# ironmanaudi/GNN-decode

Hardware: AMD Instinct MI355X
Metric: codewords/sec (whole node) at matched BER, T-iter GNN decode (higher is better)
Workload: dtype f32; 1 GPU; bch_63_45 cgnni decode, T=25, batch=65536/GPU; code=bch_63_45, model=cgnni, iters=25, global_batch=65536, parallelism=dp1 (codeword shards)

## Files before the change

### gnn-decode_amd/csrc/gnnd_common.h

```cpp
#pragma once
#include <hip/hip_runtime.h>
#include <stdint.h>
#include <math.h>
#include "../../include/gnnd.h"

#ifndef GNND_BLOCK
#define GNND_BLOCK 256
#endif

#ifdef GNND_TUNING
#include <stdlib.h>
#define gnnd_tune_env(name) getenv(name)
#else
#define gnnd_tune_env(name) ((const char*)nullptr)
#endif

enum GnndDebugBit {
    GNND_DBG_LDS_POS = 0,
    GNND_DBG_VAR = 1,
    GNND_DBG_SLOT = 2,
    GNND_DBG_NODE = 3,
    GNND_DBG_GRID = 4,
};
#ifdef GNND_DEBUG
// ... 64 lines not shown
#define GNND_PMARK(pf, i) pf.mark(i)
#define GNND_PREPORT(pf, tag, n, iters) pf.report(tag, n, iters)
#define GNND_PARG(pf, i) , &pf, i
#else
#define GNND_PPROF(pf) do { } while (0)
#define GNND_PSTART(pf, on) do { } while (0)
#define GNND_PMARK(pf, i) do { } while (0)
#define GNND_PREPORT(pf, tag, n, iters) do { } while (0)
#define GNND_PARG(pf, i)
#endif

struct GraphView {
    int V, C, E, N;
    int max_dv, max_dc;
    const uint32_t* edge_vc;
    const int* var_ptr;
    const int* chk_ptr;
    const int* chk_edge;
    int G, logG, R;
    int padded;
    int padr;
    const uint32_t* slot;
    const int* vslot;
    const uint32_t* slot_ve;
    const uint2* var_ord;
    const uint2* vlay;
    int vgroup, spare, P1;
    int ts;
    int xs, xv0, xc0, os, o0, es, e0;
};
#define GNND_SLOT_PAD 0x80000000u

struct gnnd_graph {
    GraphView view;
    GraphView rview;
    GraphView pview;
    GraphView rlay[7];
    GraphView rlayx[7];
    void* dev;
    size_t table_bytes;
    int ncomp;
    gnnd_graph* comp[8];
    GraphView* dcomp;
    int nosplit;
    int min_dc;
    int nlayers, max_layer;
    int* layer_dev;
    int* layer_of;
    int uf_nvert;
    int* uf_dev;
    int* uf_ends;
};
constexpr int kMaxComp = 8;

__host__ __device__ inline int graph_table_ints(int V, int C, int E) {
    return E + (V + 1) + (C + 1) + E;
}

int set_hip_error(hipError_t e);

#define GNND_HIP_CHECK(call)                                   \
    do {                                                       \
        hipError_t _e = (call);                                \
        if (_e != hipSuccess) return set_hip_error(_e);        \
    } while (0)

#define GNND_LAUNCH_CHECK()                                    \
    do {                                                       \
        hipError_t _e = hipGetLastError();                     \
        if (_e != hipSuccess) return set_hip_error(_e);        \
    } while (0)

struct FastDiv {
    uint32_t d, m, s;
};
inline FastDiv make_fastdiv(uint32_t d) {
    FastDiv f;
    f.d = d;
    uint32_t l = 0;
    while ((1u << l) < d) ++l;
    f.s = l;
    f.m = (uint32_t)((((uint64_t)1 << 32) * (((uint64_t)1 << l) - d)) / d + 1);
    return f;
}
__device__ __forceinline__ uint32_t fdiv(uint32_t n, const FastDiv& f) {
    return (__umulhi(n, f.m) + n) >> f.s;
}

__device__ __forceinline__ float g_tanh(float x) { return tanhf(x); }
__device__ __forceinline__ float g_log(float x) { return logf(x); }
__device__ __forceinline__ float g_exp(float x) { return expf(x); }
__device__ __forceinline__ float g_log1p(float x) { return log1pf(x); }
__device__ __forceinline__ double g_log1p(double x) { return log1p(x); }
__device__ __forceinline__ float g_cos(float x) { return cosf(x); }
__device__ __forceinline__ double g_cos(double x) { return cos(x); }
__device__ __forceinline__ float g_abs(float x) { return fabsf(x); }
__device__ __forceinline__ double g_abs(double x) { return fabs(x); }
template <typename T> __device__ __forceinline__ T g_fma(T a, T b, T c) { return fma(a, b, c); }
template <typename T> __device__ __forceinline__ T g_min(T a, T b) { return a < b ? a : b; }
template <typename T> __device__ __forceinline__ T g_max(T a, T b) { return a > b ? a : b; }
template <typename T> __device__ __forceinline__ T g_clamp(T x, T lo, T hi) {
    return x < lo ? lo : (x > hi ? hi : x);
}

__constant__ static const double kSpCoef[23] = {
    1.0 / 6227020800.0, 1.0 / 479001600.0, 1.0 / 39916800.0, 1.0 / 3628800.0,
// ... 2712 lines not shown
```

### gnn-decode_amd/csrc/gnnd_graph.hip

```cpp
#include "gnnd_common.h"
#include "gnnd_minsum_layered_host.h"
#include "gnnd_uf_host.h"
#include <stdlib.h>
#include <string.h>
#include <vector>
#include <algorithm>
#include <cmath>
#include <cstdio>

static thread_local int g_last_hip_error = 0;

int set_hip_error(hipError_t e) {
    g_last_hip_error = (int)e;
    return GNND_ERR_HIP;
}

extern "C" int gnnd_last_hip_error(void) { return g_last_hip_error; }

GNND_DEBUG_TU(graph)

extern "C" int gnnd_version(void) { return GNND_VERSION; }

extern "C" const char* gnnd_status_string(int s) {
    switch (s) {
        case GNND_OK: return "ok";
        case GNND_ERR_INVALID_ARG: return "invalid argument";
        case GNND_ERR_HIP: return "HIP runtime error";
        case GNND_ERR_UNSUPPORTED: return "unsupported configuration";
        case GNND_ERR_GRAPH: return "invalid Tanner graph (edges must be unique and sorted by (v, c))";
        case GNND_ERR_ALLOC: return "device allocation failed";
        default: return "unknown status";
    }
}

namespace {

struct SlotPlan {
    int G = 0, R = 0, padded = 0, padr = 0;
    std::vector<uint32_t> slot, slot_ve;
    std::vector<int> vslot;
};
struct Layout {
    bool ok = false;
    int P = 0;
    std::vector<int> vlay, slot;
    int ts = 0;
    std::vector<int> tpos;
};
struct HostTables {
    int V = 0, C = 0, E = 0, max_dv = 0, max_dc = 0, min_dc = 0, nints = 0, ord_off = 0, nsr = 0;
    int plan_off[3] = {0, 0, 0};
    SlotPlan plans[3];
    Layout lays[7], laysx[7];
    int lay_off[7] = {0}, layx_off[7] = {0};
    std::vector<int> table;
};

bool slot_spread_disabled() {
    static bool v = [] {
        const char* e = gnnd_tune_env("GNND_NO_SLOT_SPREAD");
        return e && e[0] == '1';
    }();
    return v;
}

void spread_check_slots(int C, int G, int R, int cw, int P, const std::vector<int>& cdeg,
                        std::vector<int>& slot) {
    const int GR = G * R, P1 = (P + 1) | 1;
    const long items = (long)C * cw * G;
    const int nh = (int)((items + 31) / 32);
    if (nh <= 0 || cw < 1) return;
    std::vector<std::vector<int>> cr_groups((size_t)C * R);
    for (int h = 0; h < nh; ++h) {
        int last = -1;
        for (int f = 32 * h; f < 32 * h + 32 && f < items; ++f) {
            const int c = (f / G) / cw;
            if (c == last) continue;
            last = c;
            for (int r = 0; r < R; ++r) cr_groups[(size_t)c * R + r].push_back(h * R + r);
        }
    }
    auto group_cost = [&](int grp) {
        const int h = grp / R, r = grp % R;
        int addr[32], n = 0;
        for (int f = 32 * h; f < 32 * h + 32 && f < items; ++f) {
            const int gi = f / G, g = f % G, c = gi / cw, b = gi % cw;
            const int k = g * R + r;
            const int pos = k < cdeg[c] ? (int)((uint32_t)slot[(size_t)c * GR + k] >> 16) : P;
            const int a = b * P1 + pos;
            bool dup = false;
            for (int i = 0; i < n && !dup; ++i) dup = addr[i] == a;
            if (!dup) addr[n++] = a;
        }
        int cnt[32] = {0}, m = 0;
        for (int i = 0; i < n; ++i) m = std::max(m, ++cnt[addr[i] & 31]);
        return m;
    };
// ... 130 lines not shown
        std::vector<int> touched, nc;
        for (long it = 0; it < iters; ++it) {
            const int a = (int)rnd(V);
            const int p2 = (int)rnd(ts);
            const int b = pos_owner[p2];
            if (b == a) continue;
            const int pa = tp[a];
            tp[a] = p2;
            if (b >= 0) tp[b] = pa;
            touched.clear();
            for (int q : of_var[a]) touched.push_back(q);
            if (b >= 0) for (int q : of_var[b]) touched.push_back(q);
            std::sort(touched.begin(), touched.end());
            touched.erase(std::unique(touched.begin(), touched.end()), touched.end());
            long delta = 0;
            nc.resize(touched.size());
            for (size_t i = 0; i < touched.size(); ++i) {
                nc[i] = cost_of(touched[i], ts, tp);
                delta += nc[i] - gc[touched[i]];
            }
            const double temp = 2.0 * (1.0 - (double)it / iters) + 0.05;
            const double u = (double)rnd(1u << 30) / (double)(1u << 30);
            if (delta <= 0 || u < exp(-(double)delta / temp)) {
                for (size_t i = 0; i < touched.size(); ++i) gc[touched[i]] = nc[i];
                cur += delta;
                pos_owner[p2] = a;
                pos_owner[pa] = b;
                if (cur < bestc) { bestc = cur; best = tp; }
            } else {
                tp[a] = pa;
                if (b >= 0) tp[b] = p2;
            }
        }
        if (best_total < 0 || bestc < best_total) {
            best_total = bestc;
            ts_out = ts;
            tpos_out = best;
        }
    }
    static const bool log = [] {
        const char* e = gnnd_tune_env("GNND_SLOT_SPREAD_LOG");
        return e && e[0] == '1';
    }();
    if (log) {
        std::vector<int> id(V);
        for (int v = 0; v < V; ++v) id[v] = v;
        long c0 = 0;
        for (int q = 0; q < ng; ++q) c0 += cost_of(q, V, id);
        fprintf(stderr, "gnnd t rows: C=%d G=%d R=%d cw=%d gather+write cycles per tile iteration "
                        "%ld (ts = V) -> %ld (ts = %d)\n", C, G, R, cw, c0, best_total, ts_out);
    }
}

int build_tables(const int64_t* h_var, const int64_t* h_chk, int64_t num_edges, int32_t V,
                 int32_t C, HostTables& T) {
    if (!h_var || !h_chk || num_edges <= 0 || V <= 0 || C <= 0) return GNND_ERR_INVALID_ARG;
    if (V > 65535 || C > 65535 || num_edges > 65535) return GNND_ERR_UNSUPPORTED;
    const int E = (int)num_edges;
    std::vector<uint32_t> evc(E);
    std::vector<int> vptr(V + 1, 0), cptr(C + 1, 0), cedge(E);
    for (int e = 0; e < E; ++e) {
        int64_t v = h_var[e], c = h_chk[e];
        if (v < 0 || v >= V || c < 0 || c >= C) return GNND_ERR_GRAPH;
        if (e > 0) {
            int64_t pv = h_var[e - 1], pc = h_chk[e - 1];
            if (v < pv || (v == pv && c <= pc)) return GNND_ERR_GRAPH;
        }
        evc[e] = (uint32_t)v | ((uint32_t)c << 16);
        vptr[v + 1]++;
        cptr[c + 1]++;
    }
    int max_dv = 0, max_dc = 0;
    for (int v = 0; v < V; ++v) { max_dv = vptr[v + 1] > max_dv ? vptr[v + 1] : max_dv; vptr[v + 1] += vptr[v]; }
    int min_dc = C > 0 ? cptr[1] : 0;
    for (int c = 0; c < C; ++c) {
        max_dc = cptr[c + 1] > max_dc ? cptr[c + 1] : max_dc;
        min_dc = cptr[c + 1] < min_dc ? cptr[c + 1] : min_dc;
        cptr[c + 1] += cptr[c];
    }
    {
        std::vector<int> fill(cptr.begin(), cptr.end() - 1);
        for (int e = 0; e < E; ++e) cedge[fill[h_chk[e]]++] = e;
    }
    static const int force_r = [] {
        const char* e = gnnd_tune_env("GNND_GROUP_R");
        return e ? atoi(e) : 0;
    }();
    auto build_plan = [&](int pref, SlotPlan& sp) -> bool {
        long best = -1;
        for (int R = 1; R <= 4; ++R) {
            int need = (max_dc + R - 1) / R, G = 1;
            while (G < need) G <<= 1;
            if (G > 64) continue;
            long slots = (long)C * G * R;
            if (force_r == R) { best = slots; sp.G = G; sp.R = R; break; }
            const bool tie_wins = pref == 1 || (pref == 2 && R == 2);
            if (best < 0 || slots < best || (tie_wins && slots == best)) {
                best = slots; sp.G = G; sp.R = R;
            }
        }
        if (best < 0) return false;
        const int ns = C * sp.G * sp.R;
        sp.slot.assign(ns, GNND_SLOT_PAD);
        sp.slot_ve.assign(ns, (uint32_t)E << 16);
        sp.vslot.assign(E, 0);
        sp.padded = 0;
        for (int c = 0; c < C; ++c) {
            sp.padded |= (cptr[c + 1] - cptr[c]) != sp.G * sp.R;
            sp.padr = std::max(sp.padr, std::min(sp.R, sp.G * sp.R - (cptr[c + 1] - cptr[c])));
            for (int k = cptr[c], i = 0; k < cptr[c + 1]; ++k, ++i) {
                int e = cedge[k];
                int pos = c * sp.G * sp.R + i;
                sp.slot[pos] = evc[e] & 0xffffu;
                sp.slot_ve[pos] = (evc[e] & 0xffffu) | ((uint32_t)e << 16);
                sp.vslot[e] = pos;
            }
        }
        return true;
    };
    SlotPlan* plans = T.plans;
    for (int i = 0; i < 3; ++i)
        if (!build_plan(i, plans[i])) return GNND_ERR_UNSUPPORTED;

    std::vector<int> vord(V);
    for (int v = 0; v < V; ++v) vord[v] = v;
    std::stable_sort(vord.begin(), vord.end(), [&](int a, int b) {
        return vptr[a + 1] - vptr[a] < vptr[b + 1] - vptr[b];
    });

    const int nints = graph_table_ints(V, C, E);
    int* plan_off = T.plan_off;
    int off = nints;
    for (int i = 0; i < 3; ++i) {
        plan_off[i] = off;
        off += 2 * (int)plans[i].slot.size() + E;
    }
    const int ord_off = (off + 1) & ~1;
    const int nsr = (int)plans[1].slot.size();
    auto build_layout = [&](int gs, bool with_x, Layout& L) {
        std::vector<int> epos(E);
        L.vlay.assign(2 * V, 0);
        int pos = 0;
        for (int j0 = 0; j0 < V; j0 += gs) {
            const int j1 = std::min(V, j0 + gs);
            int dpad = 0;
            for (int j = j0; j < j1; ++j) dpad = std::max(dpad, vptr[vord[j] + 1] - vptr[vord[j]]);
            if (with_x) ++dpad;
            for (int j = j0; j < j1; ++j) {
                const int v = vord[j];
                L.vlay[2 * j] = v | (dpad << 16);
                L.vlay[2 * j + 1] = pos;
                for (int e = vptr[v]; e < vptr[v + 1]; ++e) epos[e] = pos + (e - vptr[v]);
                pos += dpad;
            }
        }
        L.P = pos;
        if (pos >= 65535) return;
        L.ok = true;
        L.slot.assign(nsr, pos << 16);
        for (int k = 0; k < nsr; ++k) {
            const uint32_t sv = plans[1].slot_ve[k];
            const int e = (int)(sv >> 16);
            if (e < E) L.slot[k] = (int)(sv & 0xffffu) | (epos[e] << 16);
        }
        const bool tile_ok = (long)(64 / gs) * C * plans[1].G <= 12L * 256;
        if (with_x && gs >= 2 && gs <= 32 && plans[1].G <= 16 && tile_ok && !slot_spread_disabled()) {
            std::vector<int> cdeg(C);
            for (int c = 0; c < C; ++c) cdeg[c] = cptr[c + 1] - cptr[c];
            spread_check_slots(C, plans[1].G, plans[1].R, 64 / gs, pos, cdeg, L.slot);
        }
        L.ts = V;
        L.tpos.resize(V);
        for (int v = 0; v < V; ++v) L.tpos[v] = v;
        if (with_x && gs >= 2 && gs <= 32 && plans[1].G <= 16 && tile_ok && !tperm_disabled()) {
            std::vector<int> cdeg(C), vo(V);
            for (int c = 0; c < C; ++c) cdeg[c] = cptr[c + 1] - cptr[c];
            for (int j = 0; j < V; ++j) vo[j] = L.vlay[2 * j] & 0xffff;
            place_t_rows(C, plans[1].G, plans[1].R, 64 / gs, V, vo, cdeg, L.slot, L.ts, L.tpos);
        }
        if (with_x) {
            for (int j = 0; j < V; ++j) L.vlay[2 * j + 1] |= L.tpos[L.vlay[2 * j] & 0xffff] << 16;
            for (int k = 0; k < nsr; ++k)
                L.slot[k] = (L.slot[k] & ~0xffff) | L.tpos[L.slot[k] & 0xffff];
        }
    };
    Layout* lays = T.lays;
    Layout* laysx = T.laysx;
    int* lay_off = T.lay_off;
    int* layx_off = T.layx_off;
    off = ord_off + 2 * V;
    for (int i = 0; i < 7; ++i) {
        for (int x = 0; x < 2; ++x) {
            if (i == 0 && !x) continue;
            Layout& L = x ? laysx[i] : lays[i];
            build_layout(1 << i, x != 0, L);
            if (!L.ok) continue;
            (x ? layx_off : lay_off)[i] = off;
            off = (off + 2 * V + nsr + 1) & ~1;
        }
    }
    std::vector<int>& table = T.table;
    table.assign(off, 0);
    memcpy(table.data(), evc.data(), sizeof(int) * E);
    memcpy(table.data() + E, vptr.data(), sizeof(int) * (V + 1));
    memcpy(table.data() + E + V + 1, cptr.data(), sizeof(int) * (C + 1));
    memcpy(table.data() + E + V + 1 + C + 1, cedge.data(), sizeof(int) * E);
    for (int i = 0; i < 3; ++i) {
        const int ns = (int)plans[i].slot.size();
        memcpy(table.data() + plan_off[i], plans[i].slot.data(), sizeof(int) * ns);
        memcpy(table.data() + plan_off[i] + ns, plans[i].vslot.data(), sizeof(int) * E);
        memcpy(table.data() + plan_off[i] + ns + E, plans[i].slot_ve.data(), sizeof(int) * ns);
    }
    for (int i = 0; i < V; ++i) {
        const int v = vord[i];
        table[ord_off + 2 * i] = v | ((vptr[v + 1] - vptr[v]) << 16);
        table[ord_off + 2 * i + 1] = vptr[v];
    }
    for (int i = 0; i < 7; ++i)
        for (int x = 0; x < 2; ++x) {
            const Layout& L = x ? laysx[i] : lays[i];
            if (!L.ok) continue;
            const int o = (x ? layx_off : lay_off)[i];
            memcpy(table.data() + o, L.vlay.data(), sizeof(int) * 2 * V);
            memcpy(table.data() + o + 2 * V, L.slot.data(), sizeof(int) * nsr);
        }

    T.V = V; T.C = C; T.E = E; T.max_dv = max_dv; T.max_dc = max_dc; T.min_dc = min_dc;
    T.nints = nints; T.ord_off = ord_off; T.nsr = nsr;
    return GNND_OK;
}

int check_tables(const HostTables& T, int32_t* report) {
    const int E = T.E, V = T.V, C = T.C;
    const std::vector<int>& t = T.table;
    const int* vptr = t.data() + E;
    const int* cptr = vptr + V + 1;
    const int* cedge = cptr + C + 1;
    int fails = 0, nlay = 0;
    for (int p = 0; p < 3; ++p) {
        const SlotPlan& sp = T.plans[p];
        const int GR = sp.G * sp.R;
        if ((int)sp.slot_ve.size() != C * GR) { ++fails; continue; }
        for (int c = 0; c < C; ++c) {
            const int deg = cptr[c + 1] - cptr[c];
            if (deg > GR) ++fails;
            for (int i = 0; i < GR; ++i) {
                const int e = (int)(sp.slot_ve[c * GR + i] >> 16);
                if (i < deg) {
                    if (e != cedge[cptr[c] + i] || sp.vslot[e] != c * GR + i) ++fails;
                    if ((int)(sp.slot_ve[c * GR + i] & 0xffffu) != (int)(t[e] & 0xffff)) ++fails;
                } else if (e != E) {
                    ++fails;
                }
            }
            for (int gi = 0; gi < sp.G; ++gi) {
                int pad = 0;
                for (int r = 0; r < sp.R; ++r) {
                    const bool isp = (int)(sp.slot_ve[c * GR + gi * sp.R + r] >> 16) == E;
                    if (!isp && pad) ++fails;
                    pad += isp;
                }
                if (pad > sp.padr) ++fails;
            }
        }
    }
    for (int x = 0; x < 2; ++x)
        for (int i = x ? 0 : 1; i < 7; ++i) {
            const Layout& L = x ? T.laysx[i] : T.lays[i];
            if (!L.ok) continue;
            ++nlay;
            std::vector<int> owner(L.P + 1, -1), epos(E, -1);
            int expect = 0;
            const bool tx = x != 0;
            const int ts = tx ? L.ts : V;
            if (tx) {
                std::vector<int> used(ts > 0 ? ts : 1, 0);
                if ((int)L.tpos.size() != V || ts < V || ts > 65535) ++fails;
                else
                    for (int v = 0; v < V; ++v)
                        if (L.tpos[v] < 0 || L.tpos[v] >= ts || used[L.tpos[v]]++) ++fails;
            }
            auto tp = [&](int v) { return tx && (int)L.tpos.size() == V ? L.tpos[v] : v; };
            for (int j = 0; j < V; ++j) {
                const int v = L.vlay[2 * j] & 0xffff, dpad = (int)((uint32_t)L.vlay[2 * j] >> 16);
                const int pos = L.vlay[2 * j + 1] & 0xffff;
                if (((uint32_t)L.vlay[2 * j + 1] >> 16) != (uint32_t)(tx ? tp(v) : 0)) ++fails;
                const int deg = vptr[v + 1] - vptr[v];
                if (pos != expect || dpad < deg + x || pos + dpad > L.P) { ++fails; continue; }
                expect = pos + dpad;
                for (int k = 0; k < dpad; ++k) {
                    if (owner[pos + k] != -1) ++fails;
                    owner[pos + k] = v;
                }
                for (int e = vptr[v]; e < vptr[v + 1]; ++e) epos[e] = pos + (e - vptr[v]);
            }
            if (expect != L.P) ++fails;
            const SlotPlan& sp = T.plans[1];
            const int GR = sp.G * sp.R;
            std::vector<int> epos_inv(L.P + 1, -1), seen(E, 0);
            for (int e = 0; e < E; ++e)
                if (epos[e] >= 0) epos_inv[epos[e]] = e;
            for (int c = 0; c < C; ++c) {
                const int deg = cptr[c + 1] - cptr[c];
                for (int k = 0; k < GR; ++k) {
                    const uint32_t sl = (uint32_t)L.slot[c * GR + k];
                    const int pos = (int)(sl >> 16);
                    if (k >= deg) {
                        if (pos != L.P) ++fails;
                        continue;
                    }
                    const int e = pos <= L.P ? epos_inv[pos] : -1;
                    if (e < 0 || (int)(t[e] >> 16) != c || (int)(sl & 0xffffu) != tp((int)(t[e] & 0xffff)) ||
                        seen[e]++)
                        ++fails;
                }
            }
        }
    if (report) {
        report[0] = 3;
        report[1] = nlay;
        report[2] = E;
        report[3] = fails;
    }
    return fails ? GNND_ERR_GRAPH : GNND_OK;
}

}

extern "C" int gnnd_graph_validate_host(const int64_t* h_var, const int64_t* h_chk,
                                        int64_t num_edges, int32_t V, int32_t C,
                                        int32_t* h_report4) {
    HostTables T;
    const int rc = build_tables(h_var, h_chk, num_edges, V, C, T);
    if (rc != GNND_OK) return rc;
    return check_tables(T, h_report4);
}

namespace {

int create_single(const int64_t* h_var, const int64_t* h_chk, int64_t num_edges, int32_t V,
                  int32_t C, gnnd_graph** out) {
    *out = nullptr;
    HostTables T;
    const int rc = build_tables(h_var, h_chk, num_edges, V, C, T);
    if (rc != GNND_OK) return rc;
    const int E = T.E, max_dv = T.max_dv, max_dc = T.max_dc, nints = T.nints, ord_off = T.ord_off;
    const std::vector<int>& table = T.table;
    const SlotPlan* plans = T.plans;
    const Layout* lays = T.lays;
    const Layout* laysx = T.laysx;
    const int* plan_off = T.plan_off;
    const int* lay_off = T.lay_off;
    const int* layx_off = T.layx_off;
    gnnd_graph* g = (gnnd_graph*)calloc(1, sizeof(gnnd_graph));
    if (!g) return GNND_ERR_ALLOC;
    hipError_t err = hipMalloc(&g->dev, sizeof(int) * table.size());
    if (err != hipSuccess) { free(g); set_hip_error(err); return GNND_ERR_ALLOC; }
    err = hipMemcpy(g->dev, table.data(), sizeof(int) * table.size(), hipMemcpyHostToDevice);
    if (err != hipSuccess) { (void)hipFree(g->dev); free(g); return set_hip_error(err); }
    int* d = (int*)g->dev;
    g->table_bytes = sizeof(int) * (size_t)nints;
    GraphView& gv = g->view;
    gv.V = V; gv.C = C; gv.E = E; gv.N = V + C;
    gv.max_dv = max_dv; gv.max_dc = max_dc;
    gv.edge_vc = (const uint32_t*)d;
    gv.var_ptr = d + E;
    gv.chk_ptr = d + E + V + 1;
    gv.chk_edge = d + E + V + 1 + C + 1;
    gv.var_ord = (const uint2*)(d + ord_off);
    gv.xs = V + C; gv.xv0 = 0; gv.xc0 = V; gv.os = V; gv.o0 = 0; gv.es = E; gv.e0 = 0;
    gv.ts = V;
    g->ncomp = 1;
    g->min_dc = T.min_dc;
    g->rview = gv;
    g->pview = gv;
    for (int i = 0; i < 3; ++i) {
        GraphView& pv = i == 0 ? g->view : i == 1 ? g->rview : g->pview;
        const int ns = (int)plans[i].slot.size();
        pv.G = plans[i].G; pv.R = plans[i].R;
        pv.padded = plans[i].padded;
        pv.padr = plans[i].padr;
        pv.logG = 0;
        while ((1 << pv.logG) < pv.G) ++pv.logG;
        pv.slot = (const uint32_t*)(d + plan_off[i]);
        pv.vslot = d + plan_off[i] + ns;
        pv.slot_ve = (const uint32_t*)(d + plan_off[i] + ns + E);
        pv.vlay = gv.var_ord;
        pv.vgroup = 1; pv.spare = E; pv.P1 = E + 1;
    }
    for (int i = 0; i < 7; ++i) {
        for (int x = 0; x < 2; ++x) {
            GraphView& lv = x ? g->rlayx[i] : g->rlay[i];
            const Layout& L = x ? laysx[i] : lays[i];
            lv = g->rview;
            if (i == 0 && !x) continue;
            lv.vgroup = 1 << i;
            if (!L.ok) { lv.vlay = nullptr; continue; }
            const int o = (x ? layx_off : lay_off)[i];
            lv.vlay = (const uint2*)(d + o);
            lv.slot_ve = (const uint32_t*)(d + o + 2 * V);
            lv.spare = L.P;
            lv.P1 = (L.P + 1) | 1;
            lv.ts = x ? L.ts : V;
        }
    }
    {
        const int* cptr = table.data() + E + V + 1;
        const int* cedge = cptr + C + 1;
        std::vector<int> cvar(E), layer_of, layer_tab, layer_chk;
        for (int i = 0; i < E; ++i) cvar[i] = (int)((uint32_t)table[cedge[i]] & 0xffffu);
        g->nlayers = gnnd_layers_build(V, C, cptr, cvar.data(), layer_of);
        gnnd_layers_order(C, g->nlayers, layer_of, layer_tab, layer_chk);
        for (int k = 0; k < g->nlayers; ++k)
            g->max_layer = std::max(g->max_layer, layer_tab[k + 1] - layer_tab[k]);
        layer_tab.insert(layer_tab.end(), layer_chk.begin(), layer_chk.end());
        g->layer_of = (int*)malloc(sizeof(int) * (size_t)C);
        if (!g->layer_of) { (void)hipFree(g->dev); free(g); return GNND_ERR_ALLOC; }
        memcpy(g->layer_of, layer_of.data(), sizeof(int) * (size_t)C);
        err = hipMalloc((void**)&g->layer_dev, sizeof(int) * layer_tab.size());
        if (err == hipSuccess) {
            err = hipMemcpy(g->layer_dev, layer_tab.data(), sizeof(int) * layer_tab.size(),
                            hipMemcpyHostToDevice);
            if (err != hipSuccess) (void)hipFree(g->layer_dev);
        }
        if (err != hipSuccess) {
            (void)hipFree(g->dev);
            free(g->layer_of);
            free(g);
            return set_hip_error(err);
        }
    }
    *out = g;
    return GNND_OK;
}

int destroy_graph(gnnd_graph* g) {
    hipError_t err = hipSuccess;
    for (int k = 0; k < g->ncomp && g->ncomp > 1; ++k)
        if (g->comp[k]) {
            const int rc = destroy_graph(g->comp[k]);
            if (rc != GNND_OK && err == hipSuccess) err = (hipError_t)gnnd_last_hip_error();
        }
    if (g->dcomp) {
        const hipError_t e = hipFree(g->dcomp);
        if (err == hipSuccess) err = e;
    }
    const hipError_t el = hipFree(g->layer_dev);
    if (err == hipSuccess) err = el;
    free(g->layer_of);
    const hipError_t eu = hipFree(g->uf_dev);
    if (err == hipSuccess) err = eu;
    free(g->uf_ends);
    const hipError_t e = hipFree(g->dev);
    if (err == hipSuccess) err = e;
    free(g);
// ... 209 lines not shown
```

### gnn-decode_amd/gnndecode/_lib.py

```python
import ctypes
import os

_HERE = os.path.dirname(os.path.abspath(__file__))
LIB_PATH = os.environ.get('GNND_LIB') or os.path.join(_HERE, 'libgnnd.so')

OK, ERR_INVALID_ARG, ERR_HIP, ERR_UNSUPPORTED, ERR_GRAPH, ERR_ALLOC = range(6)
F32, F64, BF16 = 0, 1, 2
SOURCE_TO_TARGET, TARGET_TO_SOURCE = 0, 1
AGGR = {'add': 0, 'mean': 1, 'max': 2}
FLOW = {'source_to_target': SOURCE_TO_TARGET, 'target_to_source': TARGET_TO_SOURCE}
OSD_BASE = {'zero': 0, 'hard': 1}
OSD_METHOD = {'osd0': 0, 'cs': 1, 'e': 2}
RELAY_SOFT = {'last': 0, 'mean': 1}
BPGD_PICK = {'least': 0, 'most': 1}
VARIANT = {'v24': 0, 'qgnni': 1, 'qbp': 2, 'cgnni': 3, 'cbp': 4, 'nbp': 5, 'v10': 6, 'v30': 7, 'v22': 8}

_c_i64p = ctypes.POINTER(ctypes.c_int64)
_c_i32p = ctypes.POINTER(ctypes.c_int32)
_vp = ctypes.c_void_p
_i32 = ctypes.c_int32
_i64 = ctypes.c_int64
_int = ctypes.c_int

SIGNATURES = {
    'gnnd_graph_create': (_int, [_c_i64p, _c_i64p, _i64, _i32, _i32, ctypes.POINTER(_vp)]),
    'gnnd_graph_destroy': (_int, [_vp]),
    'gnnd_graph_validate_host': (_int, [_c_i64p, _c_i64p, _i64, _i32, _i32, _c_i32p]),
    'gnnd_graph_dims': (_int, [_vp, _c_i32p]),
    'gnnd_graph_components': (_int, [_vp, _c_i32p]),
    'gnnd_graph_set_split': (_int, [_vp, _i32]),
    'gnnd_check_tiled': (_int, [_vp, _vp, _i64, _i64, _i64, _i64, _vp, _vp]),
    'gnnd_propagate_width': (_int, [_int, _int]),
    'gnnd_propagate_tiled': (_int, [_vp, _int, _int, _int, _int, _vp, _vp, _vp, _i64, _vp]),
    'gnnd_propagate_generic_workspace': (_int, [_int, _int, _int, _int, _i64, _i64, _c_i64p]),
    'gnnd_propagate_generic': (_int, [_int, _int, _int, _int, _vp, _i64, _i64, _vp, _vp, _i64,
                                      _vp, _vp, _i64, _vp]),
    'gnnd_propagate_tiled_bwd': (_int, [_vp, _int, _int, _int, _int, _vp, _vp, _vp, _vp, _i64,
                                        _vp]),
    'gnnd_propagate_generic_bwd_workspace': (_int, [_int, _int, _int, _int, _i64, _i64, _c_i64p]),
    'gnnd_propagate_generic_bwd': (_int, [_int, _int, _int, _int, _vp, _i64, _i64, _vp, _vp, _vp,
                                          _i64, _vp, _vp, _i64, _vp]),
    'gnnd_weights_count': (_int, [_int, _c_i64p]),
    'gnnd_decode_weights_count': (_int, [_vp, _int, _i32, _c_i64p]),
    'gnnd_prepare_weights': (_int, [_int, _int, _vp, _vp, _vp]),
    'gnnd_prepared_weights_count': (_int, [_int, _int, _c_i64p]),
    'gnnd_prepared_weights_count_priors': (_int, [_int, _int, _i32, _c_i64p]),
    'gnnd_prepare_weights_priors': (_int, [_int, _int, _vp, _vp, ctypes.POINTER(ctypes.c_double), _i32,
                                           _vp]),
    'gnnd_v24_scan_priors': (_int, [_vp, _int, _vp, _i64, _vp, _vp, _vp]),
    'gnnd_prepare_weights_priors_dev': (_int, [_int, _int, _vp, _vp, _i64, _vp, _vp, _vp]),
    'gnnd_v24_var_mlp_table': (_int, [_vp, _vp, _vp, _vp, _vp, _i64, _vp]),
    'gnnd_decode': (_int, [_vp, _int, _int, _vp, _vp, _vp, _i64, _i32, _vp]),
    'gnnd_decode_tile': (_int, [_vp, _int, _int, _c_i32p, _c_i32p]),
    'gnnd_decode_plan': (_int, [_vp, _int, _int, _c_i32p]),
    'gnnd_train_tape_bytes': (_int, [_vp, _int, _int, _i64, _i32, _c_i64p]),
    'gnnd_train_fwd': (_int, [_vp, _int, _int, _vp, _vp, _vp, _vp, _i64, _i32, _vp]),
    'gnnd_train_bwd_workspace': (_int, [_vp, _int, _int, _i64, _c_i64p]),
    'gnnd_train_workspace_bytes': (_int, [_vp, _int, _int, _i64, _i32, _c_i64p]),
    'gnnd_train_bwd': (_int, [_vp, _int, _int, _vp, _vp, _vp, _vp, _vp, _vp, _vp, _i64, _i64, _i32,
                              _vp]),
    'gnnd_train_bwd_rows': (_int, [_vp, _int, _int, _i64, _c_i64p]),
    'gnnd_train_bwd_partial': (_int, [_vp, _int, _int, _vp, _vp, _vp, _vp, _vp, _vp, _i64, _i64,
                                      _i32, _vp]),
    'gnnd_train_loss_count': (_int, [_vp, _i64, _c_i64p]),
    'gnnd_train_bwd_loss_partial': (_int, [_vp, _int, _int, _vp, _vp, _vp, _vp, _vp, _i32, _i32,
                                           _vp, _vp, _vp, _i64, _i64, _i32, _vp]),
    'gnnd_train_fwd_loss': (_int, [_vp, _int, _int, _vp, _vp, _vp, _vp, _vp, _vp, _i32, _i32,
                                   _vp, _vp, _i64, _i32, _vp]),
    'gnnd_train_update': (_int, [_int, _int, _vp, _i64, _vp, _vp, _i64, _vp, _vp, _vp, _vp, _vp,
                                 _vp, ctypes.c_double, ctypes.c_double, ctypes.c_double,
                                 ctypes.c_double, ctypes.c_double, _vp, _vp]),
    'gnnd_syndrome_loss': (_int, [_vp, _vp, _i32, _i32, _int, _vp, _vp, _vp, _vp, _i64, _vp]),
    'gnnd_decision_errors': (_int, [_vp, _vp, _i32, _int, _vp, _vp, _vp, _i64, _vp]),
    'gnnd_osd0': (_int, [_vp, _int, _vp, _vp, _int, _vp, _vp, _i64, _vp]),
    'gnnd_osd0_host': (_int, [_c_i64p, _c_i64p, _i64, _i32, _i32, _int, _vp, _vp, _int, _vp, _c_i32p,
                              _i64]),
    'gnnd_osd': (_int, [_vp, _int, _vp, _vp, _int, _int, _i32, _vp, _vp, _vp, _i64, _vp]),
    'gnnd_osd_host': (_int, [_c_i64p, _c_i64p, _i64, _i32, _i32, _int, _vp, _vp, _int, _int, _i32, _vp,
                             _c_i32p, _c_i32p, _i64]),
    'gnnd_minsum': (_int, [_vp, _int, _vp, ctypes.c_double, ctypes.c_double, _i32, _i32, _vp, _vp,
# ... 147 lines not shown
```

### include/gnnd.h

```cpp
#ifndef GNND_H
#define GNND_H

#include <stdint.h>

#ifdef __cplusplus
extern "C" {
#endif

#define GNND_VERSION 1

typedef enum gnnd_status {
    GNND_OK = 0,
    GNND_ERR_INVALID_ARG = 1,
    GNND_ERR_HIP = 2,
    GNND_ERR_UNSUPPORTED = 3,
    GNND_ERR_GRAPH = 4,
    GNND_ERR_ALLOC = 5
} gnnd_status;

typedef enum gnnd_dtype { GNND_F32 = 0, GNND_F64 = 1, GNND_BF16 = 2 } gnnd_dtype;

typedef enum gnnd_flow { GNND_SOURCE_TO_TARGET = 0, GNND_TARGET_TO_SOURCE = 1 } gnnd_flow;

typedef enum gnnd_aggr { GNND_AGGR_ADD = 0, GNND_AGGR_MEAN = 1, GNND_AGGR_MAX = 2 } gnnd_aggr;

typedef enum gnnd_variant {
    GNND_V24 = 0, GNND_QGNNI = 1, GNND_QBP = 2, GNND_CGNNI = 3, GNND_CBP = 4,
    GNND_NBP = 5, GNND_V10 = 6, GNND_V30 = 7, GNND_V22 = 8
} gnnd_variant;

typedef gnnd_variant gnnd_model;

typedef struct gnnd_graph gnnd_graph;

int gnnd_graph_create(const int64_t* h_var, const int64_t* h_chk, int64_t num_edges,
                      int32_t num_var, int32_t num_chk, gnnd_graph** out);
int gnnd_graph_destroy(gnnd_graph* g);
int gnnd_graph_validate_host(const int64_t* h_var, const int64_t* h_chk, int64_t num_edges,
                             int32_t num_var, int32_t num_chk, int32_t* h_report4);
int gnnd_graph_dims(const gnnd_graph* g, int32_t* h_dims6);
int gnnd_graph_components(const gnnd_graph* g, int32_t* h_ncomp);
int gnnd_graph_set_split(gnnd_graph* g, int32_t enable);

int gnnd_check_tiled(const gnnd_graph* g, const int64_t* d_edge_index, int64_t row_stride,
                     int64_t num_batched_edges, int64_t batch, int64_t chk_shift,
                     int32_t* d_flag, void* stream);

int gnnd_propagate_width(int variant, int flow);
int gnnd_propagate_tiled(const gnnd_graph* g, int variant, int flow, int aggr, int dtype,
                         const void* d_msg, const void* d_extra, void* d_out, int64_t batch,
                         void* stream);

int gnnd_propagate_generic_workspace(int variant, int flow, int aggr, int dtype,
                                     int64_t num_edges, int64_t dim_size, int64_t* h_bytes);
int gnnd_propagate_generic(int variant, int flow, int aggr, int dtype,
                           const int64_t* d_edge_index, int64_t row_stride, int64_t num_edges,
                           const void* d_msg, const void* d_extra, int64_t dim_size,
                           void* d_out, void* d_workspace, int64_t workspace_bytes,
                           void* stream);

int gnnd_propagate_tiled_bwd(const gnnd_graph* g, int variant, int flow, int aggr, int dtype,
                             const void* d_msg, const void* d_extra, const void* d_grad_out,
                             void* d_grad_msg, int64_t batch, void* stream);
int gnnd_propagate_generic_bwd_workspace(int variant, int flow, int aggr, int dtype,
                                         int64_t num_edges, int64_t dim_size, int64_t* h_bytes);
int gnnd_propagate_generic_bwd(int variant, int flow, int aggr, int dtype,
                               const int64_t* d_edge_index, int64_t row_stride,
                               int64_t num_edges, const void* d_msg, const void* d_extra,
                               const void* d_grad_out, int64_t dim_size, void* d_grad_msg,
                               void* d_workspace, int64_t workspace_bytes, void* stream);

int gnnd_weights_count(int model, int64_t* h_count);
int gnnd_decode_weights_count(const gnnd_graph* g, int model, int32_t iters, int64_t* h_count);
int gnnd_prepare_weights(int model, int dtype, const void* d_w, void* d_prepared,
                         void* stream);
int gnnd_prepared_weights_count(int model, int dtype, int64_t* h_count);
int gnnd_decode(const gnnd_graph* g, int model, int dtype, const void* d_w, const void* d_x,
                void* d_out, int64_t batch, int32_t iters, void* stream);

int gnnd_prepared_weights_count_priors(int model, int dtype, int32_t n_priors, int64_t* h_count);
int gnnd_prepare_weights_priors(int model, int dtype, const void* d_w, void* d_prepared,
                                const double* h_priors, int32_t n_priors, void* stream);
int gnnd_v24_scan_priors(const gnnd_graph* g, int dtype, const void* d_x, int64_t batch,
                         double* d_priors, int32_t* d_status, void* stream);
int gnnd_prepare_weights_priors_dev(int model, int dtype, const void* d_w, void* d_prepared,
                                    int64_t prepared_capacity, const double* d_priors,
                                    const int32_t* d_status, void* stream);
int gnnd_v24_var_mlp_table(const void* d_w, const void* d_u, const void* d_x, void* d_y,
                           int32_t* d_hit, int64_t n, void* stream);

int gnnd_v24_check_mlp_table(const gnnd_graph* g, const void* d_w, const void* d_u, void* d_y,
                             int64_t n, int32_t* d_ok, void* stream);
// ... 256 lines not shown
```

Baseline: 146.6 million codewords/s.

## Refine LDS row placement and stride on host to reduce bank conflicts

```diff
diff --git a/gnn-decode_amd/csrc/gnnd_common.h b/gnn-decode_amd/csrc/gnnd_common.h
--- a/gnn-decode_amd/csrc/gnnd_common.h
+++ b/gnn-decode_amd/csrc/gnnd_common.h
@@ -140,6 +140,9 @@
     int* uf_ends;
 };
 constexpr int kMaxComp = 8;
+
+constexpr size_t kResidentLdsTarget = 40 * 1024;
+constexpr size_t kTxLdsFixedMax = 256 + 1024;
 
 __host__ __device__ inline int graph_table_ints(int V, int C, int E) {
     return E + (V + 1) + (C + 1) + E;
diff --git a/gnn-decode_amd/csrc/gnnd_graph.hip b/gnn-decode_amd/csrc/gnnd_graph.hip
--- a/gnn-decode_amd/csrc/gnnd_graph.hip
+++ b/gnn-decode_amd/csrc/gnnd_graph.hip
@@ -1,6 +1,7 @@
 #include "gnnd_common.h"
 #include "gnnd_minsum_layered_host.h"
 #include "gnnd_uf_host.h"
+#include "gnnd_lds_layout.h"
 #include <stdlib.h>
 #include <string.h>
 #include <vector>
@@ -43,6 +44,8 @@
 struct Layout {
     bool ok = false;
     int P = 0;
+    int P1 = 0;
+    long cost0 = -1, cost = -1;
     std::vector<int> vlay, slot;
     int ts = 0;
     std::vector<int> tpos;
@@ -279,8 +282,75 @@
     }
 }
 
+bool lds_refine_disabled() {
+    static bool v = [] {
+        const char* e = gnnd_tune_env("GNND_NO_LDS_REFINE");
+        return e && e[0] == '1';
+    }();
+    return v;
+}
+
+struct TileArrays {
+    std::vector<int> cdeg, slot_v, slot_k, vord, dpad;
+};
+gnnd_lds::Tile lds_tile(int V, int C, int G, int R, int cw, const std::vector<int>& cdeg,
+                        const Layout& L, gnnd_lds::Placement& p, TileArrays& store) {
+    const int nsr = C * G * R;
+    store.cdeg = cdeg;
+    store.slot_v.assign(nsr, 0);
+    store.slot_k.assign(nsr, 0);
+    store.vord.resize(V);
+    store.dpad.resize(V);
+    p.ts = L.ts;
+    p.P1 = L.P1;
+    p.spare = L.P;
+    p.tpos = L.tpos;
+    p.rbase.assign(V, 0);
+    for (int j = 0; j < V; ++j) {
+        const int v = L.vlay[2 * j] & 0xffff;
+        store.vord[j] = v;
+        store.dpad[j] = (int)((uint32_t)L.vlay[2 * j] >> 16);
+        p.rbase[v] = L.vlay[2 * j + 1] & 0xffff;
+    }
+    for (int c = 0; c < C; ++c)
+        for (int k = 0; k < cdeg[c] && k < G * R; ++k) {
+            const uint32_t s = (uint32_t)L.slot[(size_t)c * G * R + k];
+            store.slot_v[(size_t)c * G * R + k] = (int)(s & 0xffffu);
+            store.slot_k[(size_t)c * G * R + k] = (int)(s >> 16) - p.rbase[s & 0xffffu];
+        }
+    gnnd_lds::Tile t;
+    t.V = V; t.C = C; t.G = G; t.R = R; t.cw = cw; t.block = GNND_BLOCK;
+    t.cdeg = store.cdeg.data();
+    t.slot_v = store.slot_v.data();
+    t.slot_k = store.slot_k.data();
+    t.vord = store.vord.data();
+    t.dpad = store.dpad.data();
+    return t;
+}
+
+void refine_lds(int V, int C, int G, int R, int cw, const std::vector<int>& cdeg, Layout& L) {
+    gnnd_lds::Placement p;
+    TileArrays store;
+    const gnnd_lds::Tile t = lds_tile(V, C, G, R, cw, cdeg, L, p, store);
+    const long avail = (long)kResidentLdsTarget - (long)kTxLdsFixedMax - (((long)V * 8 + 15) & ~15L) -
+                       8 - 4L * cw * C;
+    long extra = (avail - 4L * cw * ((long)L.P1 + L.ts)) / (4L * cw);
+    extra = std::max(0L, std::min(extra, (long)gnnd_lds::kBanks));
+    while (extra > 0 && (long)cw * (L.P1 + extra) >= 65536) --extra;
+    L.cost = gnnd_lds::refine_placement(t, p, (int)extra, &L.cost0);
+    if (L.cost >= L.cost0) return;
+    L.P1 = p.P1;
+    L.tpos = p.tpos;
+    for (int j = 0; j < V; ++j) L.vlay[2 * j + 1] = p.rbase[store.vord[j]];
+    for (int c = 0; c < C; ++c)
+        for (int k = 0; k < cdeg[c] && k < G * R; ++k) {
+            const size_t i = (size_t)c * G * R + k;
+            L.slot[i] = store.slot_v[i] | ((p.rbase[store.slot_v[i]] + store.slot_k[i]) << 16);
+        }
+}
+
 int build_tables(const int64_t* h_var, const int64_t* h_chk, int64_t num_edges, int32_t V,
-                 int32_t C, HostTables& T) {
+                 int32_t C, HostTables& T, bool refine_off = false) {
     if (!h_var || !h_chk || num_edges <= 0 || V <= 0 || C <= 0) return GNND_ERR_INVALID_ARG;
     if (V > 65535 || C > 65535 || num_edges > 65535) return GNND_ERR_UNSUPPORTED;
     const int E = (int)num_edges;
@@ -382,6 +452,7 @@
             }
         }
         L.P = pos;
+        L.P1 = (pos + 1) | 1;
         if (pos >= 65535) return;
         L.ok = true;
         L.slot.assign(nsr, pos << 16);
@@ -404,6 +475,18 @@
             for (int c = 0; c < C; ++c) cdeg[c] = cptr[c + 1] - cptr[c];
             for (int j = 0; j < V; ++j) vo[j] = L.vlay[2 * j] & 0xffff;
             place_t_rows(C, plans[1].G, plans[1].R, 64 / gs, V, vo, cdeg, L.slot, L.ts, L.tpos);
+        }
+        if (with_x && gs >= 2 && gs <= 32 && plans[1].G <= 16 && tile_ok && GNND_BLOCK % (64 / gs) == 0) {
+            std::vector<int> cdeg(C);
+            for (int c = 0; c < C; ++c) cdeg[c] = cptr[c + 1] - cptr[c];
+            if (!lds_refine_disabled() && !refine_off)
+                refine_lds(V, C, plans[1].G, plans[1].R, 64 / gs, cdeg, L);
+            else {
+                gnnd_lds::Placement p;
+                TileArrays store;
+                L.cost = L.cost0 = gnnd_lds::model_cost(
+                    lds_tile(V, C, plans[1].G, plans[1].R, 64 / gs, cdeg, L, p, store), p);
+            }
         }
         if (with_x) {
             for (int j = 0; j < V; ++j) L.vlay[2 * j + 1] |= L.tpos[L.vlay[2 * j] & 0xffff] << 16;
@@ -497,7 +580,8 @@
             if (!L.ok) continue;
             ++nlay;
             std::vector<int> owner(L.P + 1, -1), epos(E, -1);
-            int expect = 0;
+            int covered = 0;
+            if (L.P1 <= L.P || L.P1 > 65535) ++fails;
             const bool tx = x != 0;
             const int ts = tx ? L.ts : V;
             if (tx) {
@@ -513,15 +597,15 @@
                 const int pos = L.vlay[2 * j + 1] & 0xffff;
                 if (((uint32_t)L.vlay[2 * j + 1] >> 16) != (uint32_t)(tx ? tp(v) : 0)) ++fails;
                 const int deg = vptr[v + 1] - vptr[v];
-                if (pos != expect || dpad < deg + x || pos + dpad > L.P) { ++fails; continue; }
-                expect = pos + dpad;
+                if (dpad < deg + x || pos + dpad > L.P) { ++fails; continue; }
+                covered += dpad;
                 for (int k = 0; k < dpad; ++k) {
                     if (owner[pos + k] != -1) ++fails;
                     owner[pos + k] = v;
                 }
                 for (int e = vptr[v]; e < vptr[v + 1]; ++e) epos[e] = pos + (e - vptr[v]);
             }
-            if (expect != L.P) ++fails;
+            if (covered != L.P) ++fails;
             const SlotPlan& sp = T.plans[1];
             const int GR = sp.G * sp.R;
             std::vector<int> epos_inv(L.P + 1, -1), seen(E, 0);
@@ -561,6 +645,66 @@
     const int rc = build_tables(h_var, h_chk, num_edges, V, C, T);
     if (rc != GNND_OK) return rc;
     return check_tables(T, h_report4);
+}
+
+extern "C" int gnnd_graph_lds_layout_host(const int64_t* h_var, const int64_t* h_chk,
+                                          int64_t num_edges, int32_t V, int32_t C, int32_t cw,
+                                          int32_t refine, int32_t* h_report8, int32_t* h_vlay,
+                                          int32_t* h_slot, int32_t* h_tpos) {
+    int i = 0;
+    while (i < 7 && (cw << i) != 64) ++i;
+    if (cw < 2 || i < 1 || i > 5 || !h_report8) return GNND_ERR_INVALID_ARG;
+    HostTables T;
+    const int rc = build_tables(h_var, h_chk, num_edges, V, C, T, refine == 0);
+    if (rc != GNND_OK) return rc;
+    const Layout& L = T.laysx[i];
+    if (!L.ok || L.cost < 0) return GNND_ERR_UNSUPPORTED;
+    const int32_t rep[8] = {T.plans[1].G, T.plans[1].R, L.P, L.P1, L.ts, T.nsr,
+                            (int32_t)L.cost0, (int32_t)L.cost};
+    memcpy(h_report8, rep, sizeof(rep));
+    if (h_vlay) memcpy(h_vlay, L.vlay.data(), sizeof(int) * 2 * (size_t)V);
+    if (h_slot) memcpy(h_slot, L.slot.data(), sizeof(int) * (size_t)T.nsr);
+    if (h_tpos) memcpy(h_tpos, L.tpos.data(), sizeof(int) * (size_t)V);
+    return GNND_OK;
+}
+
+extern "C" int gnnd_lds_model_cost_host(int32_t V, int32_t C, int32_t G, int32_t R, int32_t cw,
+                                        const int32_t* cdeg, const int32_t* slot_v,
+                                        const int32_t* slot_k, const int32_t* vord,
+                                        const int32_t* dpad, const int32_t* rbase,
+                                        const int32_t* tpos, int32_t ts, int32_t P1, int32_t spare,
+                                        int64_t* h_cost3) {
+    if (V < 1 || C < 1 || G < 1 || R < 1 || cw < 1 || cw > GNND_BLOCK || GNND_BLOCK % cw || !cdeg ||
+        !slot_v || !slot_k || !vord || !dpad || !rbase || !tpos || !h_cost3 || ts < V || ts > 65535 ||
+        spare < 0 || P1 <= spare || P1 > 65535 || (long)C * cw * G > 64L * GNND_BLOCK)
+        return GNND_ERR_INVALID_ARG;
+    std::vector<char> row(ts, 0);
+    for (int v = 0; v < V; ++v) {
+        if (tpos[v] < 0 || tpos[v] >= ts || row[tpos[v]]++) return GNND_ERR_INVALID_ARG;
+        if (vord[v] < 0 || vord[v] >= V || dpad[v] < 1 || rbase[v] < 0 || rbase[v] + dpad[v] > 65535)
+            return GNND_ERR_INVALID_ARG;
+    }
+    for (int c = 0; c < C; ++c) {
+        if (cdeg[c] < 0 || cdeg[c] > G * R) return GNND_ERR_INVALID_ARG;
+        for (int k = 0; k < cdeg[c]; ++k) {
+            const size_t i = (size_t)c * G * R + k;
+            if (slot_v[i] < 0 || slot_v[i] >= V || slot_k[i] < 0 || slot_k[i] > 65535)
+                return GNND_ERR_INVALID_ARG;
+        }
+    }
+    gnnd_lds::Tile t;
+    t.V = V; t.C = C; t.G = G; t.R = R; t.cw = cw; t.block = GNND_BLOCK;
+    t.cdeg = cdeg; t.slot_v = slot_v; t.slot_k = slot_k; t.vord = vord; t.dpad = dpad;
+    gnnd_lds::Placement p;
+    p.ts = ts; p.P1 = P1; p.spare = spare;
+    p.tpos.assign(tpos, tpos + V);
+    p.rbase.assign(rbase, rbase + V);
+    gnnd_lds::Space Ts, Ms;
+    gnnd_lds::build_spaces(t, p, Ts, Ms);
+    h_cost3[0] = Ts.total;
+    h_cost3[1] = Ms.total;
+    h_cost3[2] = Ts.total + Ms.total;
+    return GNND_OK;
 }
 
 namespace {
@@ -627,7 +771,7 @@
             lv.vlay = (const uint2*)(d + o);
             lv.slot_ve = (const uint32_t*)(d + o + 2 * V);
             lv.spare = L.P;
-            lv.P1 = (L.P + 1) | 1;
+            lv.P1 = L.P1;
             lv.ts = x ? L.ts : V;
         }
     }
diff --git a/gnn-decode_amd/csrc/gnnd_lds_layout.h b/gnn-decode_amd/csrc/gnnd_lds_layout.h
--- /dev/null
+++ b/gnn-decode_amd/csrc/gnnd_lds_layout.h
@@ -0,0 +1,214 @@
+#pragma once
+#include <algorithm>
+#include <cstdint>
+#include <vector>
+
+namespace gnnd_lds {
+
+constexpr int kBanks = 32;
+constexpr int kGroupLanes = 32;
+
+inline int extra_passes(int* addr, int n) {
+    if (n <= 1) return 0;
+    std::sort(addr, addr + n);
+    int cnt[kBanks] = {0}, m = 0;
+    for (int i = 0; i < n; ++i)
+        if (i == 0 || addr[i] != addr[i - 1]) m = std::max(m, ++cnt[addr[i] % kBanks]);
+    return m - 1;
+}
+
+struct Tile {
+    int V = 0, C = 0, G = 1, R = 1, cw = 1, block = 256;
+    const int* cdeg = nullptr;
+    const int* slot_v = nullptr;
+    const int* slot_k = nullptr;
+    const int* vord = nullptr;
+    const int* dpad = nullptr;
+};
+
+struct Placement {
+    int ts = 0, P1 = 0, spare = 0;
+    std::vector<int> tpos;
+    std::vector<int> rbase;
+};
+
+struct Space {
+    struct Lane { int b, var, off; };
+    int stride = 0;
+    std::vector<int> base;
+    std::vector<int> len;
+    std::vector<Lane> lanes;
+    std::vector<int> gstart{0};
+    std::vector<int> gcost;
+    std::vector<std::vector<int>> of_var;
+    long total = 0;
+
+    void end_group() {
+        if ((int)lanes.size() > gstart.back()) gstart.push_back((int)lanes.size());
+    }
+    int group_cost(int q) const {
+        int addr[kGroupLanes], n = 0;
+        for (int i = gstart[q]; i < gstart[q + 1]; ++i)
+            addr[n++] = lanes[i].b * stride + base[lanes[i].var] + lanes[i].off;
+        return extra_passes(addr, n);
+    }
+    void index() {
+        const int ng = (int)gstart.size() - 1;
+        of_var.assign(base.size(), {});
+        for (int q = 0; q < ng; ++q)
+            for (int i = gstart[q]; i < gstart[q + 1]; ++i) {
+                std::vector<int>& o = of_var[lanes[i].var];
+                if (o.empty() || o.back() != q) o.push_back(q);
+            }
+        recost();
+    }
+    void recost() {
+        const int ng = (int)gstart.size() - 1;
+        gcost.resize(ng);
+        total = 0;
+        for (int q = 0; q < ng; ++q) total += gcost[q] = group_cost(q);
+    }
+    long try_swap(int a, int b, std::vector<int>& touched) {
+        touched.clear();
+        touched.insert(touched.end(), of_var[a].begin(), of_var[a].end());
+        touched.insert(touched.end(), of_var[b].begin(), of_var[b].end());
+        std::sort(touched.begin(), touched.end());
+        touched.erase(std::unique(touched.begin(), touched.end()), touched.end());
+        std::swap(base[a], base[b]);
+        long delta = 0;
+        for (int q : touched) delta += group_cost(q) - gcost[q];
+        if (delta >= 0) {
+            std::swap(base[a], base[b]);
+            return 0;
+        }
+        for (int q : touched) gcost[q] = group_cost(q);
+        total += delta;
+        return -delta;
+    }
+    void refine(long max_evals) {
+        const int n = (int)base.size();
+        std::vector<int> touched;
+        long evals = 0;
+        for (int sweep = 0; sweep < 4 && evals < max_evals; ++sweep) {
+            bool improved = false;
+            for (int a = 0; a < n && evals < max_evals; ++a) {
+                bool hot = false;
+                for (int q : of_var[a]) hot = hot || gcost[q] > 0;
+                if (!hot) continue;
+                uint32_t seen = 0;
+                for (int d = 1; d < n && evals < max_evals; ++d) {
+                    const int b = (a + d) % n;
+                    if (len[b] != len[a]) continue;
+                    const int res = base[b] % kBanks;
+                    if (res == base[a] % kBanks || ((seen >> res) & 1u)) continue;
+                    seen |= 1u << res;
+                    ++evals;
+                    if (try_swap(a, b, touched) > 0) { improved = true; seen = 0; }
+                }
+            }
+            if (!improved) break;
+        }
+    }
+};
+
+inline void build_spaces(const Tile& t, const Placement& p, Space& T, Space& M) {
+    const int V = t.V, C = t.C, G = t.G, R = t.R, cw = t.cw, GR = G * R;
+    T = Space();
+    M = Space();
+    T.stride = p.ts;
+    T.base.assign(p.tpos.begin(), p.tpos.end());
+    {
+        std::vector<char> used(p.ts > 0 ? p.ts : 1, 0);
+        for (int v = 0; v < V; ++v) used[p.tpos[v]] = 1;
+        for (int r = 0; r < p.ts; ++r)
+            if (!used[r]) T.base.push_back(r);
+    }
+    T.len.assign(T.base.size(), 1);
+    M.stride = p.P1;
+    M.base.assign(p.rbase.begin(), p.rbase.end());
+    M.base.push_back(p.spare);
+    M.len.assign(V + 1, 0);
+    for (int i = 0; i < V; ++i) M.len[t.vord[i]] = t.dpad[i];
+    const long items = (long)C * cw * G;
+    const int Q = (int)((items + t.block - 1) / t.block);
+    for (int q = 0; q < Q; ++q)
+        for (int h = 0; h < t.block / kGroupLanes; ++h)
+            for (int r = 0; r < R; ++r) {
+                for (int l = 0; l < kGroupLanes; ++l) {
+                    const long f = (long)q * t.block + h * kGroupLanes + l;
+                    const int gi = (int)(f / G), g = (int)(f % G), c = gi / cw, b = gi % cw;
+                    const int cc = c < C ? c : C - 1, k = g * R + r;
+                    const bool real = k < t.cdeg[cc];
+                    const int v = real ? t.slot_v[(size_t)cc * GR + k] : 0;
+                    T.lanes.push_back({b, v, 0});
+                    if (real && c < C) M.lanes.push_back({b, v, t.slot_k[(size_t)cc * GR + k]});
+                    else M.lanes.push_back({b, V, 0});
+                }
+                T.end_group();
+                M.end_group();
+            }
+    if (t.block % cw == 0) {
+        const int vstep = t.block / cw;
+        for (int i0 = 0; i0 < V; i0 += vstep)
+            for (int h = 0; h < t.block / kGroupLanes; ++h) {
+                int dp = 0;
+                for (int l = 0; l < kGroupLanes; ++l) {
+                    const int i = i0 + (h * kGroupLanes + l) / cw;
+                    if (i < V) dp = std::max(dp, t.dpad[i]);
+                }
+                for (int k = 0; k < dp; ++k) {
+                    for (int l = 0; l < kGroupLanes; ++l) {
+                        const int tid = h * kGroupLanes + l, i = i0 + tid / cw;
+                        if (i < V && k < t.dpad[i]) M.lanes.push_back({tid % cw, t.vord[i], k});
+                    }
+                    M.end_group();
+                }
+                for (int l = 0; l < kGroupLanes; ++l) {
+                    const int tid = h * kGroupLanes + l, i = i0 + tid / cw;
+                    if (i < V) T.lanes.push_back({tid % cw, t.vord[i], 0});
+                }
+                T.end_group();
+            }
+    }
+    T.index();
+    M.index();
+}
+
+inline long model_cost(const Tile& t, const Placement& p) {
+    Space T, M;
+    build_spaces(t, p, T, M);
+    return T.total + M.total;
+}
+
+constexpr long kMaxEvals = 1500;
+
+inline long refine_placement(const Tile& t, Placement& p, int extra_p1, long* parent_cost = nullptr) {
+    Space T, M;
+    build_spaces(t, p, T, M);
+    const long cost0 = T.total + M.total;
+    if (parent_cost) *parent_cost = cost0;
+    auto best_stride = [&]() {
+        int best = M.stride;
+        long bc = M.total;
+        for (int s = p.P1; s <= p.P1 + extra_p1; ++s) {
+            M.stride = s;
+            M.recost();
+            if (M.total < bc) { bc = M.total; best = s; }
+        }
+        M.stride = best;
+        M.recost();
+    };
+    best_stride();
+    M.refine(kMaxEvals);
+    best_stride();
+    T.refine(kMaxEvals);
+    if (T.total + M.total >= cost0) return cost0;
+    p.P1 = M.stride;
+    for (int v = 0; v < t.V; ++v) {
+        p.tpos[v] = T.base[v];
+        p.rbase[v] = M.base[v];
+    }
+    return T.total + M.total;
+}
+
+}
diff --git a/gnn-decode_amd/gnndecode/_lib.py b/gnn-decode_amd/gnndecode/_lib.py
--- a/gnn-decode_amd/gnndecode/_lib.py
+++ b/gnn-decode_amd/gnndecode/_lib.py
@@ -26,6 +26,9 @@
     'gnnd_graph_create': (_int, [_c_i64p, _c_i64p, _i64, _i32, _i32, ctypes.POINTER(_vp)]),
     'gnnd_graph_destroy': (_int, [_vp]),
     'gnnd_graph_validate_host': (_int, [_c_i64p, _c_i64p, _i64, _i32, _i32, _c_i32p]),
+    'gnnd_graph_lds_layout_host': (_int, [_c_i64p, _c_i64p, _i64, _i32, _i32, _i32, _i32, _c_i32p,
+                                          _c_i32p, _c_i32p, _c_i32p]),
+    'gnnd_lds_model_cost_host': (_int, [_i32] * 5 + [_c_i32p] * 7 + [_i32] * 3 + [_c_i64p]),
     'gnnd_graph_dims': (_int, [_vp, _c_i32p]),
     'gnnd_graph_components': (_int, [_vp, _c_i32p]),
     'gnnd_graph_set_split': (_int, [_vp, _i32]),
diff --git a/include/gnnd.h b/include/gnnd.h
--- a/include/gnnd.h
+++ b/include/gnnd.h
@@ -38,6 +38,15 @@
 int gnnd_graph_destroy(gnnd_graph* g);
 int gnnd_graph_validate_host(const int64_t* h_var, const int64_t* h_chk, int64_t num_edges,
                              int32_t num_var, int32_t num_chk, int32_t* h_report4);
+int gnnd_graph_lds_layout_host(const int64_t* h_var, const int64_t* h_chk, int64_t num_edges,
+                               int32_t num_var, int32_t num_chk, int32_t cw, int32_t refine,
+                               int32_t* h_report8, int32_t* h_vlay, int32_t* h_slot,
+                               int32_t* h_tpos);
+int gnnd_lds_model_cost_host(int32_t V, int32_t C, int32_t G, int32_t R, int32_t cw,
+                             const int32_t* cdeg, const int32_t* slot_v, const int32_t* slot_k,
+                             const int32_t* vord, const int32_t* dpad, const int32_t* rbase,
+                             const int32_t* tpos, int32_t ts, int32_t P1, int32_t spare,
+                             int64_t* h_cost3);
 int gnnd_graph_dims(const gnnd_graph* g, int32_t* h_dims6);
 int gnnd_graph_components(const gnnd_graph* g, int32_t* h_ncomp);
 int gnnd_graph_set_split(gnnd_graph* g, int32_t enable);
```

New measurement: 147.9 million codewords/s, median of 6. No clear change (+0.9%).
